# GDMCF/GDMCF

Hardware: AMD Instinct MI355X
Metric: training users/sec (higher is better)
Workload: dtype f32; 1 GPU; yelp-shape synthetic rows, batch=400/GPU, dims=[1000], T=5, noise_scale=0.01, linear-var, mean_type=x0, reweight, AdamW lr=1e-5 (BASELINE configs[1]); n_items=34395, global_batch=400, parallelism=dp1, batch_rows=device CSR rows (CsrBatch)

## Files before the change

### gdmcf_amd/csrc/gemm_dr.h

```cpp
#pragma once

#include "common.h"

namespace {
struct DrArgs {
    GdGemm g;
    int tiles_m, tiles_n, m_fastest;
    int ksp;
    int ctr;
    const GdAdamHyper* adam_dev;
    int stagger;
};
}

struct DrRoutes {
    bool dw;
    bool adamw;
    bool kn;
    bool fat;
    bool fat_slab;
};
DrRoutes& dr_routes();
int dr_cu_count();
int dr_stagger();

int gd_dr_tn_launch(GdGemm& g, hipStream_t s);
int gd_dr_kn_launch(GdGemm& g, hipStream_t s);
int gd_dr_fat_launch(int epi, GdGemm& g, hipStream_t s);
int gd_dr_fat_slab_launch(GdGemm& g, hipStream_t s);
```

### gdmcf_amd/csrc/gemm_dr_fat.hip

```cpp
#include <stdlib.h>

#include "gemm_dr.h"

#ifndef GD_FAT_DMA_DEFAULT
#define GD_FAT_DMA_DEFAULT 1
#endif

namespace {

template <int NB, int EPI, int DMA>
__global__ __launch_bounds__(256, 1) void dr_fat_kernel(const DrArgs d) {
    static_assert(EPI == GD_EPI_LOSS || EPI == GD_EPI_POST || EPI == GD_EPI_SLAB, "output layer with a fused epilogue, or split-K slabs");
    static_assert(NB >= 4 && NB <= 12, "5 x NB accumulator blocks must fit 256 registers");
    static_assert(DMA == 0 || DMA == 1, "B through staging registers, or straight into LDS");
    constexpr bool SLAB = EPI == GD_EPI_SLAB;
    typedef __attribute__((address_space(3))) void* lds_vp;
    constexpr int WAIT_VM0 = 0x0F70, WAIT_LGKM0 = 0xC07F;
    constexpr int TMB = 5;
    const GdGemm& g = d.g;
    const int lane = threadIdx.x & 63;
    const int wave = __builtin_amdgcn_readfirstlane(threadIdx.x >> 6);
    const int r = lane & 15, q = lane >> 4;
    extern __shared__ __attribute__((aligned(16))) float dr_lds[];
    float* const lds = dr_lds + wave * (2 * NB * 256);
    const int nblk = gridDim.x, per = nblk >> 3;
    const int wl = ((nblk & 7) == 0 ? ((int)(blockIdx.x & 7) * per + (int)(blockIdx.x >> 3)) : (int)blockIdx.x) * 4 + wave;
    const int n_waves = nblk * 4;
    const int ntiles = d.tiles_m * d.tiles_n;
    const __amdgpu_buffer_rsrc_t srdA = __builtin_amdgcn_make_buffer_rsrc(const_cast<float*>(g.A), 0, (int)(((int64_t)(g.M - 1) * g.lda + g.K) * 4), 0x00020000);
    const __amdgpu_buffer_rsrc_t srdB = __builtin_amdgcn_make_buffer_rsrc(const_cast<float*>(g.B), 0, (int)(((int64_t)(g.N - 1) * g.ldb + g.K) * 4), 0x00020000);
    const int NCH = d.ksp;
    const int c_mask = g.K >> 4;
    const int ntasks = SLAB ? ntiles * g.splits : ntiles;
    const int w_off = (lane >> 2) * 16 + (((lane & 3) ^ ((((lane >> 2) >> 2) & 1) << 1)) << 2);
    const int g_slot = DMA ? ((lane & 3) ^ ((((lane >> 2) >> 2) & 1) << 1)) : (lane & 3);
    const int r_off = r * 16 + ((q ^ (((r >> 2) & 1) << 1)) << 2);
    for (int task = wl; task < ntasks; task += n_waves) {
        const int split = SLAB ? task / ntiles : 0;
        const int tile = SLAB ? task - split * ntiles : task;
        const int c_lo = SLAB ? split * (g.kchunk >> 4) : 0;
        const int c_hi = SLAB ? min(c_lo + (g.kchunk >> 4), NCH) : NCH;
        const int c_in = SLAB ? min(c_hi, c_mask) : c_mask;
        const int tm = tile % d.tiles_m, tn = tile / d.tiles_m;
        const int m0 = tm * (16 * TMB), n0 = tn * (16 * NB);
        uint32_t offA[TMB], offB[NB];
#pragma unroll
        for (int i = 0; i < TMB; ++i) offA[i] = (uint32_t)((m0 + 16 * i + r) * g.lda + 4 * q) * 4u;
#pragma unroll
        for (int p = 0; p < NB; ++p) offB[p] = (uint32_t)(((int64_t)(n0 + 16 * p + (lane >> 2)) * g.ldb + 4 * g_slot) * 4);
        f32x4 acc[TMB][NB];
#pragma unroll
        for (int i = 0; i < TMB; ++i)
#pragma unroll
            for (int b = 0; b < NB; ++b) acc[i][b] = f32x4{0.f, 0.f, 0.f, 0.f};
        f32x4 xa[2][TMB], G[DMA ? 1 : NB], FB[NB];
        const int hp = DMA ? ((c_in - c_lo) & 1) : 0;
        const int k_lo = SLAB ? c_lo * 64 : 0;
        if (hp) {
#pragma unroll
            for (int i = 0; i < TMB; ++i) xa[1][i] = __builtin_bit_cast(f32x4, __builtin_amdgcn_raw_buffer_load_b128(srdA, offA[i], k_lo, 0));
        } else {
#pragma unroll
            for (int i = 0; i < TMB; ++i) xa[0][i] = __builtin_bit_cast(f32x4, __builtin_amdgcn_raw_buffer_load_b128(srdA, offA[i], k_lo, 0));
        }
        if constexpr (DMA) {
            __builtin_amdgcn_sched_barrier(0);
            __builtin_amdgcn_s_waitcnt(WAIT_LGKM0);
            __builtin_amdgcn_sched_barrier(0);
#pragma unroll
            for (int p = 0; p < NB; ++p) __builtin_amdgcn_raw_ptr_buffer_load_lds(srdB, (lds_vp)(lds + hp * (NB * 256) + p * 256), 16, (int)offB[p], k_lo, 0, 0);
        } else {
#pragma unroll
            for (int p = 0; p < NB; ++p) G[p] = __builtin_bit_cast(f32x4, __builtin_amdgcn_raw_buffer_load_b128(srdB, offB[p], k_lo, 0));
#pragma unroll
            for (int p = 0; p < NB; ++p) *reinterpret_cast<f32x4*>(lds + p * 256 + w_off) = G[p];
        }

#define GD_FAT_CHUNK(PAR, c, MSK)                                                                                         \
        {                                                                                                             \
             \
            const uint32_t kn = ((c) + 1 < c_hi) ? (uint32_t)((c) + 1) * 64u : 0x80000000u;                           \
            if constexpr (DMA) {                                                                                      \
                __builtin_amdgcn_sched_barrier(0);                                                                    \
                __builtin_amdgcn_s_waitcnt(WAIT_VM0);                                                                 \
                __builtin_amdgcn_sched_barrier(0);                                                                    \
            }                                                                                                         \
            _Pragma("unroll") for (int b = 0; b < NB; ++b)                                                            \
                FB[b] = *reinterpret_cast<const f32x4*>(lds + (PAR) * (NB * 256) + b * 256 + r_off);                  \
            if (MSK) {  \
                 \
                _Pragma("unroll") for (int e = 0; e < 4; ++e) {                                                       \
                    const bool keep = (c) * 16 + 4 * q + e < g.K;                                                     \
                    _Pragma("unroll") for (int i = 0; i < TMB; ++i) xa[PAR][i][e] = keep ? xa[PAR][i][e] : 0.f;       \
                    _Pragma("unroll") for (int b = 0; b < NB; ++b) FB[b][e] = keep ? FB[b][e] : 0.f;                  \
                }                                                                                                     \
            }                                                                                                         \
            __builtin_amdgcn_sched_barrier(0);                                                                        \
            _Pragma("unroll") for (int sx = 0; sx < 4; ++sx) {                                                        \
                _Pragma("unroll") for (int n = 0; n < TMB * NB; ++n) {                                                \
                    const int i = n / NB, b = n % NB;                                                                 \
                    if (sx == 0 && i == 0) asm volatile("" : "+v"(FB[b]));  \
                    if (sx == 0 && b == 0) asm volatile("" : "+v"(xa[PAR][i]));                                       \
                    acc[i][b] = __builtin_amdgcn_mfma_f32_16x16x4f32(xa[PAR][i][sx], FB[b][sx], acc[i][b], 0, 0, 0);  \
                     \
                    if (sx < 2 && n % 5 == 2) {      \
                        const int l = (sx == 0) ? n / 5 : NB + n / 5;                                                 \
                        if (l < TMB + NB) {                                                                           \
                            __builtin_amdgcn_sched_barrier(0);                                                        \
                            if (l < TMB)                                                                              \
                                xa[(PAR) ^ 1][l] = __builtin_bit_cast(f32x4, __builtin_amdgcn_raw_buffer_load_b128(   \
                                    srdA, offA[l], kn, 0));                                                           \
                            else if constexpr (DMA)                                                                   \
                                __builtin_amdgcn_raw_ptr_buffer_load_lds(                                             \
                                    srdB, (lds_vp)(lds + ((PAR) ^ 1) * (NB * 256) + (l - TMB) * 256), 16,             \
                                    (int)offB[l - TMB], (int)kn, 0, 0);                                               \
                            else                                                                                      \
                                G[l - TMB] = __builtin_bit_cast(f32x4, __builtin_amdgcn_raw_buffer_load_b128(         \
                                    srdB, offB[l - TMB], kn, 0));                                                     \
                            __builtin_amdgcn_sched_barrier(0);                                                        \
                        }                                                                                             \
                    }                                                                                                 \
                    if (!DMA && sx == 3 && n % 4 == 1 && n / 4 < NB) {  \
                        __builtin_amdgcn_sched_barrier(0);                                                            \
                        *reinterpret_cast<f32x4*>(lds + ((PAR) ^ 1) * (NB * 256) + (n / 4) * 256 + w_off) = G[n / 4]; \
                        __builtin_amdgcn_sched_barrier(0);                                                            \
                    }                                                                                                 \
                }                                                                                                     \
                __builtin_amdgcn_sched_barrier(0);                                                                    \
            }                                                                                                         \
        }
        const int c_pf = d.stagger > 0 ? ((NCH > d.stagger + 2 ? NCH - d.stagger : 0) & ~1) : -2;
        const int c_pairs = DMA ? c_in : c_hi;
        const int c_pfl = (DMA && c_pf >= 0) ? min(c_pf | hp, c_pairs - 2) : c_pf;
        int c = c_lo;
        if constexpr (DMA) {
            if (hp) {
                GD_FAT_CHUNK(1, c_lo, false);
                c = c_lo + 1;
            }
        }
        for (; c + 1 < c_pairs; c += 2) {
            if constexpr (EPI == GD_EPI_POST) {
                if (c == c_pfl) {
                    constexpr int NJL = (16 * NB * 4 + 127) / 128 + 1;
                    constexpr int NPI = (80 * NJL + 63) / 64;
                    float* const scratch = dr_lds + 4 * (2 * NB * 256) + wave * 64;
                    const __amdgpu_buffer_rsrc_t srdX = __builtin_amdgcn_make_buffer_rsrc(
                        const_cast<float*>(g.aux), 0, (int)(((int64_t)(g.M - 1) * g.ldaux + g.N) * 4), 0x00020000);
#pragma unroll
                    for (int pi = 0; pi < NPI; ++pi) {
                        const int t = min(pi * 64 + lane, 80 * NJL - 1);
                        const int row = min(m0 + t % 80, g.M - 1), j = t / 80;
                        const int col = min(j < NJL - 1 ? n0 + 32 * j : n0 + 16 * NB - 1, g.N - 1);
                        __builtin_amdgcn_raw_ptr_buffer_load_lds(srdX, (lds_vp)scratch, 4, (int)(((int64_t)row * g.ldaux + col) * 4), 0, 0, 0);
                    }
                }
            }
            if constexpr (DMA) {
                GD_FAT_CHUNK(0, c, false);
                GD_FAT_CHUNK(1, c + 1, false);
            } else {
                GD_FAT_CHUNK(0, c, c >= c_mask);
                GD_FAT_CHUNK(1, c + 1, c + 1 >= c_mask);
            }
        }
        if constexpr (DMA) {
            if (c < c_hi) GD_FAT_CHUNK(0, c, true);
        } else {
            if ((c_hi - c_lo) & 1) GD_FAT_CHUNK(0, c_hi - 1, c_hi - 1 >= c_mask);
        }
#undef GD_FAT_CHUNK
        if constexpr (DMA) {
            __builtin_amdgcn_sched_barrier(0);
            __builtin_amdgcn_s_waitcnt(WAIT_VM0);
            __builtin_amdgcn_sched_barrier(0);
        }

        if constexpr (SLAB) {
            constexpr int LDS_S = 16 * NB + 4, NJ_S = (4 * NB + 15) / 16;
            float* const slab = g.C + (int64_t)split * g.slab_stride;
#pragma unroll
            for (int i = 0; i < TMB; ++i) {
#pragma unroll
                for (int b = 0; b < NB; ++b)
#pragma unroll
                    for (int t = 0; t < 4; ++t) lds[(4 * q + t) * LDS_S + 16 * b + r] = acc[i][b][t];
                __builtin_amdgcn_sched_barrier(0);
#pragma unroll
                for (int p4 = 0; p4 < 4; ++p4) {
                    const int m = m0 + 16 * i + 4 * p4 + q;
#pragma unroll
                    for (int j = 0; j < NJ_S; ++j) {
                        const int c4 = r + 16 * j;
                        const int n = n0 + 4 * c4;
                        const f32x4 v = *reinterpret_cast<const f32x4*>(lds + (4 * p4 + q) * LDS_S + 4 * min(c4, 4 * NB - 1));
                        if (c4 < 4 * NB && m < g.M) {
                            if (n + 3 < g.N) {
                                *reinterpret_cast<f32x4*>(slab + (int64_t)m * g.ldc + n) = v;
                            } else {
                                for (int e = 0; e < 4 && n + e < g.N; ++e) slab[(int64_t)m * g.ldc + n + e] = v[e];
                            }
                        }
                    }
                }
                __builtin_amdgcn_sched_barrier(0);
            }
            continue;
        }

        constexpr int LDS_ = 16 * NB + 4;
        constexpr int NJ = (4 * NB + 15) / 16;
        typedef f32x4 f32x4_e __attribute__((aligned(4)));
        f32x4 bias4[NJ];
        int col4[NJ];
#pragma unroll
        for (int j = 0; j < NJ; ++j) {
            col4[j] = n0 + 4 * (r + 16 * j);
            bias4[j] = f32x4{0.f, 0.f, 0.f, 0.f};
            if (g.bias && r + 16 * j < 4 * NB) {
#pragma unroll
                for (int e = 0; e < 4; ++e) bias4[j][e] = g.bias[min(col4[j] + e, g.N - 1)];
            }
        }
        const bool has_z = (EPI == GD_EPI_POST) && (g.aux2 != nullptr);
        const bool has_r = (EPI == GD_EPI_POST) && (g.r2 != nullptr);
        struct Pre {
            f32x4 a[NJ], z[NJ];
            uint32_t w[NJ];
            float c1, c2, p1, p2, sg;
        } pre[2];
        auto fetch = [&](int i, int p4, Pre& P) {
            const int mc = min(m0 + 16 * i + 4 * p4 + q, g.M - 1);
            P.c1 = 1.f; P.c2 = 0.f; P.p1 = 0.f; P.p2 = 0.f; P.sg = 0.f;
            if (EPI == GD_EPI_LOSS) {
                if (g.r0) P.c1 = g.r0[mc];
            } else {
                P.c1 = g.r0[mc];
                P.c2 = g.r1[mc];
                if (has_r) { P.p1 = g.r2[mc]; P.p2 = g.r3[mc]; }
                if (has_z) P.sg = g.r4[mc];
            }
#pragma unroll
            for (int j = 0; j < NJ; ++j) {
                const int n = col4[j];
                const bool whole = (r + 16 * j < 4 * NB) && n + 3 < g.N;
                P.w[j] = 0u;
                P.a[j] = f32x4{0.f, 0.f, 0.f, 0.f};
                P.z[j] = f32x4{0.f, 0.f, 0.f, 0.f};
                if (EPI == GD_EPI_LOSS && g.aux_bits) {
                    P.w[j] = g.aux_bits[(int64_t)mc * g.ldbits + min((int64_t)(n >> 5), g.ldbits - 1)];
                } else if (whole) {
                    P.a[j] = *reinterpret_cast<const f32x4_e*>(g.aux + (int64_t)mc * g.ldaux + n);
                    if (has_z) P.z[j] = *reinterpret_cast<const f32x4_e*>(g.aux2 + (int64_t)mc * g.ldaux2 + n);
                }
            }
        };
        fetch(0, 0, pre[0]);
#pragma unroll
        for (int i = 0; i < TMB; ++i) {
#pragma unroll
            for (int b = 0; b < NB; ++b)
#pragma unroll
                for (int t = 0; t < 4; ++t) lds[(4 * q + t) * LDS_ + 16 * b + r] = acc[i][b][t];
            __builtin_amdgcn_sched_barrier(0);
#pragma unroll
            for (int p4 = 0; p4 < 4; ++p4) {
                const int step = 4 * i + p4;
                const Pre& P = pre[step & 1];
                if (step + 1 < 4 * TMB) fetch((step + 1) >> 2, (step + 1) & 3, pre[(step + 1) & 1]);
                const int m = m0 + 16 * i + 4 * p4 + q;
                const int mc = min(m, g.M - 1);
                const bool mok = m < g.M;
                float ss = 0.f;
                const float c1 = P.c1, c2 = P.c2, p1 = P.p1, p2 = P.p2, sg = P.sg;
#pragma unroll
                for (int j = 0; j < NJ; ++j) {
                    const int c4 = r + 16 * j;
                    const bool inb = c4 < 4 * NB;
                    const int n = col4[j];
                    const bool whole = inb && n + 3 < g.N;
                    const bool full = whole && mok;
                    const f32x4 v = *reinterpret_cast<const f32x4*>(lds + (4 * p4 + q) * LDS_ + 4 * min(c4, 4 * NB - 1));
                    f32x4 o, o2 = f32x4{0.f, 0.f, 0.f, 0.f};
                    if (EPI == GD_EPI_LOSS) {
                        f32x4 tg;
                        if (g.aux_bits) {
                            const uint32_t w = P.w[j] >> (n & 31);
#pragma unroll
                            for (int e = 0; e < 4; ++e) tg[e] = (float)((w >> e) & 1u);
                        } else if (whole) {
                            tg = P.a[j];
                        } else {
#pragma unroll
                            for (int e = 0; e < 4; ++e) tg[e] = g.aux[(int64_t)mc * g.ldaux + min(n + e, g.N - 1)];
                        }
#pragma unroll
                        for (int e = 0; e < 4; ++e) {
                            o2[e] = v[e] + bias4[j][e];
                            o[e] = c1 * o2[e] - tg[e];
                            if (inb && mok && n + e < g.N) ss += o[e] * o[e];
                        }
                    } else {
                        f32x4 xt = P.a[j], zz = P.z[j];
                        if (!whole) {
#pragma unroll
                            for (int e = 0; e < 4; ++e) {
                                xt[e] = g.aux[(int64_t)mc * g.ldaux + min(n + e, g.N - 1)];
                                if (has_z) zz[e] = g.aux2[(int64_t)mc * g.ldaux2 + min(n + e, g.N - 1)];
                            }
                        }
#pragma unroll
                        for (int e = 0; e < 4; ++e) {
                            const float vv = v[e] + bias4[j][e];
                            o2[e] = has_r ? (p1 * xt[e] - p2 * vv) : vv;
                            o[e] = c1 * o2[e] + c2 * xt[e];
                            if (has_z) o[e] += sg * zz[e];
                        }
                    }
                    if (full) {
                        *reinterpret_cast<f32x4_e*>(g.C + (int64_t)m * g.ldc + n) = o;
                        if (g.out2) *reinterpret_cast<f32x4_e*>(g.out2 + (int64_t)m * g.ldout2 + n) = o2;
                    } else if (inb && mok) {
                        for (int e = 0; e < 4 && n + e < g.N; ++e) {
                            g.C[(int64_t)m * g.ldc + n + e] = o[e];
                            if (g.out2) g.out2[(int64_t)m * g.ldout2 + n + e] = o2[e];
                        }
                    }
                }
                if (EPI == GD_EPI_LOSS) {
                    ss += __shfl_xor(ss, 1);
                    ss += __shfl_xor(ss, 2);
                    ss += __shfl_xor(ss, 4);
                    ss += __shfl_xor(ss, 8);
                    if (r == 0 && mok) g.rowpart[(int64_t)m * g.ld_rowpart + tn] = ss;
                }
                __builtin_amdgcn_sched_barrier(0);
            }
        }
    }
}

template <int NB>
int dr_fat_go(const DrArgs& d, int epi, int dma, int n_cu, hipStream_t s) {
    const size_t lds = (size_t)4 * 2 * NB * 256 * sizeof(float) + 4 * 64 * sizeof(float);
    void (*kern)(const DrArgs) =
        dma ? (epi == GD_EPI_SLAB ? dr_fat_kernel<NB, GD_EPI_SLAB, 1> : epi == GD_EPI_LOSS ? dr_fat_kernel<NB, GD_EPI_LOSS, 1> : dr_fat_kernel<NB, GD_EPI_POST, 1>)
            : (epi == GD_EPI_SLAB ? dr_fat_kernel<NB, GD_EPI_SLAB, 0> : epi == GD_EPI_LOSS ? dr_fat_kernel<NB, GD_EPI_LOSS, 0> : dr_fat_kernel<NB, GD_EPI_POST, 0>);
    static bool attr_set[6] = {false, false, false, false, false, false};
    const int ai = epi == GD_EPI_SLAB ? 4 + dma : 2 * dma + (epi == GD_EPI_LOSS);
    if (!attr_set[ai] && lds > 48 * 1024) {
        hipError_t e = hipFuncSetAttribute(reinterpret_cast<const void*>(kern), hipFuncAttributeMaxDynamicSharedMemorySize, (int)lds);
        if (e != hipSuccess) {
            gdmcf_set_error("hipFuncSetAttribute(dr_fat_kernel, LDS=%zu): %s", lds, hipGetErrorString(e));
            return GDMCF_E_HIP;
        }
        attr_set[ai] = true;
    }
    hipLaunchKernelGGL(kern, dim3(n_cu), dim3(256), lds, s, d);
    return GDMCF_OK;
}

int dr_fat_dma(const GdGemm& g) {
    static const int dma_env = getenv("GDMCF_FAT_DMA") ? atoi(getenv("GDMCF_FAT_DMA")) : GD_FAT_DMA_DEFAULT;
    return (dma_env > 0 && (reinterpret_cast<uintptr_t>(g.B) & 15) == 0 && (g.ldb & 3) == 0) ? 1 : 0;
}

}

int gd_dr_fat_launch(int epi, GdGemm& g, hipStream_t s) {
    if (!dr_routes().fat) return GD_DR_NOT_TAKEN;
    const int64_t lim = (int64_t)1 << 32;
    const int n_cu = dr_cu_count();
    const int tiles_m = gd_cdiv(g.M, 80);
    bool ok = (int64_t)g.M * g.lda * 4 < ((int64_t)1 << 31) && (int64_t)g.N * g.ldb * 4 < lim && g.lda >= g.K && g.ldb >= g.K &&
              g.K >= 256 && (long)tiles_m * 80 * 100 <= (long)g.M * 112 &&
              (n_cu & 7) == 0 && !(epi == GD_EPI_LOSS && g.rowpart == nullptr) &&
              !(epi == GD_EPI_LOSS && g.aux_bits && g.ldbits < (g.N + 31) / 32);
    int nb = 0;
    long best = 1L << 60;
    const long slots = 4L * n_cu;
    for (int c = 12; c >= 8 && ok; --c) {
        const long t = (long)tiles_m * gd_cdiv(g.N, 16 * c);
        const long cost = ((t + slots - 1) / slots) * c;
        if (t >= slots / 2 && cost < best) { best = cost; nb = c; }
    }
    if (ok && epi == GD_EPI_POST) {
        const long t128 = (long)gd_cdiv(g.M, 80) * gd_cdiv(g.N, 128);
        const long rounds = (t128 + 2 * n_cu - 1) / (2 * n_cu);
        if (t128 * 100 >= rounds * 2 * n_cu * 90) ok = false;
    }
    if (!ok || !nb || (epi == GD_EPI_LOSS && g.ld_rowpart < gd_cdiv(g.N, 16 * nb))) return GD_DR_NOT_TAKEN;
    DrArgs d = {};
    d.tiles_m = tiles_m;
    d.tiles_n = gd_cdiv(g.N, 16 * nb);
    d.m_fastest = 1;
    d.ksp = gd_cdiv(g.K, 16);
    {
        static const int pf = getenv("GDMCF_FAT_PF") ? atoi(getenv("GDMCF_FAT_PF")) : 10;
        d.stagger = pf;
    }
    const int dma = dr_fat_dma(g);
    g.tiles_m = d.tiles_m;
    g.tiles_n = d.tiles_n;
    d.g = g;
    d.ctr = 0;
    int rc = GDMCF_OK;
    {
        GdProfScope prof(g.prof_tag, 2.0 * g.M * g.N * g.K, s);
        switch (nb) {
            case 8: rc = dr_fat_go<8>(d, epi, dma, n_cu, s); break;
            case 9: rc = dr_fat_go<9>(d, epi, dma, n_cu, s); break;
            case 10: rc = dr_fat_go<10>(d, epi, dma, n_cu, s); break;
            case 11: rc = dr_fat_go<11>(d, epi, dma, n_cu, s); break;
            default: rc = dr_fat_go<12>(d, epi, dma, n_cu, s); break;
        }
    }
    if (rc != GDMCF_OK) return rc;
    t_gd_last_gemm = 4;
    return gd_launch_status("gemm_dr");
}

int gd_dr_fat_slab_plan(int M, int N, int K, int* nb_out, int* cps_out) {
    if (!dr_routes().fat_slab || M <= 0 || N < 128 || K < 4096) return 0;
    const int n_cu = dr_cu_count();
    const int tiles_m = gd_cdiv(M, 80);
    if ((n_cu & 7) != 0 || (long)tiles_m * 80 * 100 > (long)M * 112) return 0;
    const long slots = 4L * n_cu;
    const int chunks = gd_cdiv(K, 16);
    int nb = 0, cps = 0;
    long best = 1L << 60;
    for (int c = 8; c <= 12; ++c) {
        const long tiles = (long)tiles_m * gd_cdiv(N, 16 * c);
        if (tiles > slots) continue;
        long sp = slots / tiles;
        if (sp > chunks / 8) sp = chunks / 8;
        if (sp > 64) sp = 64;
        if (sp < 2) continue;
        const int per = gd_cdiv(chunks, (int)sp);
        if ((long)c * per < best) { best = (long)c * per; nb = c; cps = per; }
    }
    if (!nb) return 0;
    if (nb_out) *nb_out = nb;
    if (cps_out) *cps_out = cps;
    return gd_cdiv(chunks, cps);
}

int gd_dr_fat_slab_launch(GdGemm& g, hipStream_t s) {
    int nb = 0, cps = 0;
    const int splits = gd_dr_fat_slab_plan(g.M, g.N, g.K, &nb, &cps);
    if (!splits) return GD_DR_NOT_TAKEN;
    const size_t need = (size_t)splits * g.M * g.ldc * sizeof(float);
    const bool ok = gd_aligned16(g.C) && (g.ldc & 3) == 0 && g.ldc >= g.N &&
                    g.ws_cap >= need && g.slab_stride >= (int64_t)g.M * g.ldc && (g.slab_stride & 3) == 0 &&
                    (int64_t)g.M * g.lda * 4 < ((int64_t)1 << 31) && (int64_t)g.N * g.ldb * 4 < ((int64_t)1 << 32) && g.lda >= g.K && g.ldb >= g.K;
    if (!ok) return GD_DR_NOT_TAKEN;
    const int n_cu = dr_cu_count();
    DrArgs d = {};
    d.tiles_m = gd_cdiv(g.M, 80);
    d.tiles_n = gd_cdiv(g.N, 16 * nb);
    d.m_fastest = 1;
    d.ksp = gd_cdiv(g.K, 16);
    g.splits = splits;
    g.kchunk = cps * 16;
    g.tiles_m = d.tiles_m;
    g.tiles_n = d.tiles_n;
    d.g = g;
    d.ctr = 0;
    const int dma = dr_fat_dma(g);
    int rc = GDMCF_OK;
    {
        GdProfScope prof(g.prof_tag, 2.0 * g.M * g.N * g.K, s);
        switch (nb) {
            case 8: rc = dr_fat_go<8>(d, GD_EPI_SLAB, dma, n_cu, s); break;
            case 9: rc = dr_fat_go<9>(d, GD_EPI_SLAB, dma, n_cu, s); break;
            case 10: rc = dr_fat_go<10>(d, GD_EPI_SLAB, dma, n_cu, s); break;
            case 11: rc = dr_fat_go<11>(d, GD_EPI_SLAB, dma, n_cu, s); break;
            default: rc = dr_fat_go<12>(d, GD_EPI_SLAB, dma, n_cu, s); break;
        }
    }
    if (rc != GDMCF_OK) return rc;
    t_gd_last_gemm = 6;
    return gd_launch_status("gemm_dr_fat_slab");
}
```

Before: 322,500 users/s.

## Add lean buffer-load epilogue variants to the fat output-layer GEMM kernel

Adds a specialized epilogue for the fat GEMM's fused loss and post-processing outputs. It reads the GdGemm fields from the kernarg segment, uses raw buffer loads and stores with out-of-range parking offsets in place of branches and bounds clamps, and increments offsets by strides. The aim is to cut scalar and vector instruction overhead, register pressure and divergent guarded stores in the epilogue, which runs after the 34k-wide output GEMM. It adds template instantiations per variant, a special path for the ragged last column tile, 32-bit offset limits checked on the host, and debug switches.

```diff
diff --git a/gdmcf_amd/csrc/gemm_dr.h b/gdmcf_amd/csrc/gemm_dr.h
--- a/gdmcf_amd/csrc/gemm_dr.h
+++ b/gdmcf_amd/csrc/gemm_dr.h
@@ -24,6 +24,7 @@
 int dr_cu_count();
 int dr_stagger();
 
+
 int gd_dr_tn_launch(GdGemm& g, hipStream_t s);
 int gd_dr_kn_launch(GdGemm& g, hipStream_t s);
 int gd_dr_fat_launch(int epi, GdGemm& g, hipStream_t s);
diff --git a/gdmcf_amd/csrc/gemm_dr_fat.hip b/gdmcf_amd/csrc/gemm_dr_fat.hip
--- a/gdmcf_amd/csrc/gemm_dr_fat.hip
+++ b/gdmcf_amd/csrc/gemm_dr_fat.hip
@@ -5,12 +5,235 @@
 #ifndef GD_FAT_DMA_DEFAULT
 #define GD_FAT_DMA_DEFAULT 1
 #endif
+#ifndef GD_FAT_EPI_DEFAULT
+#define GD_FAT_EPI_DEFAULT 1
+#endif
+#ifndef GD_FAT_EPI_DBG
+#define GD_FAT_EPI_DBG 0
+#endif
 
 namespace {
 
-template <int NB, int EPI, int DMA>
+template <int NB, int EPI, int VAR>
+__device__ __forceinline__ void dr_fat_lean_epilogue(f32x4 (&acc)[5][NB], float* const lds, const int m0, const int n0, const int tn,
+                                                     const bool last_tn, int r, int q) {
+#pragma clang fp contract(off)
+    static_assert(offsetof(DrArgs, g) == 0, "the lean epilogue finds its GdGemm at offset 0 of the kernel-argument segment");
+    typedef const __attribute__((address_space(4))) DrArgs* kargs_p;
+    kargs_p ka = (kargs_p)__builtin_amdgcn_kernarg_segment_ptr();
+    asm volatile("" : "+s"(ka), "+v"(r), "+v"(q));
+    const __attribute__((address_space(4))) GdGemm& g = ka->g;
+    constexpr int TMB = 5, LDS_ = 16 * NB + 4, NJ = (4 * NB + 15) / 16;
+    constexpr bool LOSS = EPI == GD_EPI_LOSS, BITS = LOSS && VAR == 1, GEN = !LOSS && VAR == 2;
+    constexpr bool NO_ST = (GD_FAT_EPI_DBG & 2) != 0;
+    constexpr uint32_t PARK = 0x80000000u;
+    typedef uint32_t u32x4 __attribute__((ext_vector_type(4)));
+    auto srd = [](const void* p, int64_t bytes) {
+        return __builtin_amdgcn_make_buffer_rsrc(const_cast<void*>(p), 0, p ? (int)bytes : 0, 0x00020000);
+    };
+    auto ld1 = [](__amdgpu_buffer_rsrc_t s, uint32_t off) { return __builtin_amdgcn_raw_buffer_load_b32(s, (int)off, 0, 0); };
+    auto ld1f = [](__amdgpu_buffer_rsrc_t s, uint32_t off) { return __builtin_bit_cast(float, __builtin_amdgcn_raw_buffer_load_b32(s, (int)off, 0, 0)); };
+    auto ld4f = [](__amdgpu_buffer_rsrc_t s, uint32_t off) { return __builtin_bit_cast(f32x4, __builtin_amdgcn_raw_buffer_load_b128(s, (int)off, 0, 0)); };
+    auto st1f = [](float v, __amdgpu_buffer_rsrc_t s, uint32_t off) { __builtin_amdgcn_raw_buffer_store_b32(__builtin_bit_cast(uint32_t, v), s, (int)off, 0, 0); };
+    auto st4f = [](f32x4 v, __amdgpu_buffer_rsrc_t s, uint32_t off) { __builtin_amdgcn_raw_buffer_store_b128(__builtin_bit_cast(u32x4, v), s, (int)off, 0, 0); };
+    const int M = g.M, N = g.N;
+    const bool has_o2 = g.out2 != nullptr;
+    const bool has_r = GEN && g.r2 != nullptr, has_z = GEN && g.aux2 != nullptr;
+    const __amdgpu_buffer_rsrc_t srdC = srd(NO_ST ? nullptr : g.C, ((int64_t)(M - 1) * g.ldc + N) * 4);
+    const __amdgpu_buffer_rsrc_t srdO = srd(NO_ST ? nullptr : g.out2, ((int64_t)(M - 1) * g.ldout2 + N) * 4);
+    const __amdgpu_buffer_rsrc_t srdP = srd(NO_ST || !LOSS ? nullptr : g.rowpart, ((int64_t)(M - 1) * g.ld_rowpart + g.tiles_n) * 4);
+    const __amdgpu_buffer_rsrc_t srdBias = srd(g.bias, (int64_t)N * 4);
+    const __amdgpu_buffer_rsrc_t srdR0 = srd(g.r0, (int64_t)M * 4);
+    const __amdgpu_buffer_rsrc_t srdR1 = srd(LOSS ? nullptr : g.r1, (int64_t)M * 4);
+    const __amdgpu_buffer_rsrc_t srdR2 = srd(has_r ? g.r2 : nullptr, (int64_t)M * 4);
+    const __amdgpu_buffer_rsrc_t srdR3 = srd(has_r ? g.r3 : nullptr, (int64_t)M * 4);
+    const __amdgpu_buffer_rsrc_t srdR4 = srd(has_z ? g.r4 : nullptr, (int64_t)M * 4);
+    const __amdgpu_buffer_rsrc_t srdT = BITS ? srd(g.aux_bits, (int64_t)M * g.ldbits * 4) : srd(g.aux, ((int64_t)(M - 1) * g.ldaux + N) * 4);
+    const __amdgpu_buffer_rsrc_t srdZ = srd(has_z ? g.aux2 : nullptr, ((int64_t)(M - 1) * g.ldaux2 + N) * 4);
+
+    const uint32_t row = (uint32_t)(m0 + q), col = (uint32_t)(n0 + 4 * r);
+    uint32_t offC = (row * (uint32_t)g.ldc + col) * 4u, offO = (row * (uint32_t)g.ldout2 + col) * 4u;
+    uint32_t offP = (row * (uint32_t)g.ld_rowpart + (uint32_t)tn) * 4u;
+    uint32_t offT = BITS ? (row * (uint32_t)g.ldbits + (col >> 5)) * 4u : (row * (uint32_t)g.ldaux + col) * 4u;
+    uint32_t offZ = (row * (uint32_t)g.ldaux2 + col) * 4u;
+    const uint32_t strC = (uint32_t)g.ldc * 16u, strO = (uint32_t)g.ldout2 * 16u, strP = (uint32_t)g.ld_rowpart * 16u;
+    const uint32_t strT = (BITS ? (uint32_t)g.ldbits : (uint32_t)g.ldaux) * 16u, strZ = (uint32_t)g.ldaux2 * 16u;
+    const uint32_t offR = row * 4u;
+    const uint32_t sh = col & 31u;
+    bool gok[NJ];
+    f32x4 bias4[NJ];
+#pragma unroll
+    for (int j = 0; j < NJ; ++j) {
+        gok[j] = (r + 16 * j < 4 * NB) && (n0 + 4 * (r + 16 * j) + 3 < N);
+        bias4[j] = ld4f(srdBias, (gok[j] ? col * 4u : PARK) + 256u * j);
+    }
+    const bool sedge = last_tn && (N & 3) != 0;
+    const int c4s = sedge ? ((N - 1 - n0) >> 2) : 0;
+    const int ne = N & 3;
+    const uint32_t ns = (uint32_t)(n0 + 4 * c4s);
+    const bool sl = sedge && r == (c4s & 15);
+    const uint32_t dCs = (ns - col) * 4u;
+    const uint32_t dTs = BITS ? ((ns >> 5) - (col >> 5)) * 4u : dCs;
+    uint32_t parkS[3], dE[3];
+    float bs[3] = {0.f, 0.f, 0.f};
+#pragma unroll
+    for (int e = 0; e < 3; ++e) {
+        parkS[e] = (sl && e < ne) ? 0u : PARK;
+        dE[e] = 4u * (uint32_t)min(e, max(ne - 1, 0));
+    }
+    if (sedge) {
+#pragma unroll
+        for (int e = 0; e < 3; ++e) bs[e] = ld1f(srdBias, ns * 4u + dE[e]);
+    }
+
+    struct Pre {
+        f32x4 a[NJ], z[NJ];
+        uint32_t w[NJ], ws;
+        float c1, c2, p1, p2, sg, sa[3], sz[3];
+    } pre[2];
+    auto fetch = [&](const int step, Pre& P) {
+        const uint32_t oR = offR + 16u * step;
+        if constexpr (LOSS) {
+            const float c = ld1f(srdR0, oR);
+            P.c1 = g.r0 ? c : 1.f;
+        } else {
+            P.c1 = ld1f(srdR0, oR);
+            P.c2 = ld1f(srdR1, oR);
+            if constexpr (GEN) {
+                P.p1 = ld1f(srdR2, oR);
+                P.p2 = ld1f(srdR3, oR);
+                P.sg = ld1f(srdR4, oR);
+            }
+        }
+#pragma unroll
+        for (int j = 0; j < NJ; ++j) {
+            if constexpr (BITS) {
+                P.w[j] = ld1(srdT, offT + 8u * j);
+            } else {
+                P.a[j] = ld4f(srdT, (gok[j] ? offT : PARK) + 256u * j);
+                if constexpr (GEN) P.z[j] = ld4f(srdZ, (gok[j] ? offZ : PARK) + 256u * j);
+            }
+        }
+        if (sedge) {
+            if constexpr (BITS) {
+                P.ws = ld1(srdT, offT + dTs);
+            } else {
+#pragma unroll
+                for (int e = 0; e < 3; ++e) {
+                    P.sa[e] = ld1f(srdT, offT + dTs + dE[e]);
+                    if constexpr (GEN) P.sz[e] = ld1f(srdZ, offZ + dCs + dE[e]);
+                }
+            }
+        }
+    };
+    auto elem = [&](const Pre& P, float v, float b, float t, float z, float& o2, float& o) {
+        const float vv = v + b;
+        if constexpr (LOSS) {
+            o2 = vv;
+            o = __builtin_fmaf(P.c1, vv, -t);
+        } else {
+            o2 = vv;
+            if constexpr (GEN) {
+                const float e0 = P.p1 * t, e1 = P.p2 * vv;
+                o2 = has_r ? e0 - e1 : vv;
+            }
+            const float c = P.c1 * o2;
+            o = __builtin_fmaf(P.c2, t, c);
+            if constexpr (GEN) o = has_z ? __builtin_fmaf(P.sg, z, o) : o;
+        }
+    };
+    fetch(0, pre[0]);
+#pragma unroll
+    for (int i = 0; i < TMB; ++i) {
+#pragma unroll
+        for (int b = 0; b < NB; ++b)
+#pragma unroll
+            for (int t = 0; t < 4; ++t) lds[(4 * q + t) * LDS_ + 16 * b + r] = acc[i][b][t];
+        __builtin_amdgcn_sched_barrier(0);
+#pragma unroll
+        for (int p4 = 0; p4 < 4; ++p4) {
+            const int step = 4 * i + p4;
+            const Pre& P = pre[step & 1];
+            if (step + 1 < 4 * TMB) {
+                offT += strT;
+                if constexpr (GEN) offZ += strZ;
+                fetch(step + 1, pre[(step + 1) & 1]);
+            }
+            const float* const lrow = lds + (4 * p4 + q) * LDS_;
+            float ss = 0.f;
+            f32x4 o2s[NJ];
+#pragma unroll
+            for (int j = 0; j < NJ; ++j) {
+                const f32x4 v = *reinterpret_cast<const f32x4*>(lrow + 4 * r + 64 * j);
+                f32x4 t, z = f32x4{0.f, 0.f, 0.f, 0.f}, o;
+                if constexpr (BITS) {
+                    const uint32_t w = P.w[j] >> sh;
+#pragma unroll
+                    for (int e = 0; e < 4; ++e) t[e] = (float)((w >> e) & 1u);
+                } else {
+                    t = P.a[j];
+                    if constexpr (GEN) z = P.z[j];
+                }
+                float s2 = ss;
+#pragma unroll
+                for (int e = 0; e < 4; ++e) {
+                    float o2e, oe;
+                    elem(P, v[e], bias4[j][e], t[e], z[e], o2e, oe);
+                    o2s[j][e] = o2e;
+                    o[e] = oe;
+                    if constexpr (LOSS) {
+                        const float sq = oe * oe;
+                        s2 = s2 + sq;
+                    }
+                }
+                if constexpr (LOSS) ss = gok[j] ? s2 : ss;
+                st4f(o, srdC, (gok[j] ? offC : PARK) + 256u * j);
+            }
+            if (has_o2) {
+#pragma unroll
+                for (int j = 0; j < NJ; ++j) st4f(o2s[j], srdO, (gok[j] ? offO : PARK) + 256u * j);
+            }
+            if (sedge) {
+                const f32x4 v = *reinterpret_cast<const f32x4*>(lrow + 4 * c4s);
+                float s2 = ss;
+#pragma unroll
+                for (int e = 0; e < 3; ++e) {
+                    float t, z = 0.f, o2, o;
+                    if constexpr (BITS) {
+                        t = (float)((P.ws >> ((ns & 31u) + e)) & 1u);
+                    } else {
+                        t = P.sa[e];
+                        if constexpr (GEN) z = P.sz[e];
+                    }
+                    elem(P, v[e], bs[e], t, z, o2, o);
+                    if constexpr (LOSS) {
+                        const float sq = o * o;
+                        s2 = (e < ne) ? s2 + sq : s2;
+                    }
+                    st1f(o, srdC, (offC + dCs + 4u * e) | parkS[e]);
+                    if (has_o2) st1f(o2, srdO, (offO + dCs + 4u * e) | parkS[e]);
+                }
+                if constexpr (LOSS) ss = sl ? s2 : ss;
+            }
+            if constexpr (LOSS) {
+                ss += __shfl_xor(ss, 1);
+                ss += __shfl_xor(ss, 2);
+                ss += __shfl_xor(ss, 4);
+                ss += __shfl_xor(ss, 8);
+                st1f(ss, srdP, r == 0 ? offP : PARK);
+                offP += strP;
+            }
+            offC += strC;
+            offO += strO;
+            __builtin_amdgcn_sched_barrier(0);
+        }
+    }
+}
+
+template <int NB, int EPI, int DMA, int VAR>
 __global__ __launch_bounds__(256, 1) void dr_fat_kernel(const DrArgs d) {
     static_assert(EPI == GD_EPI_LOSS || EPI == GD_EPI_POST || EPI == GD_EPI_SLAB, "output layer with a fused epilogue, or split-K slabs");
+    static_assert(VAR >= 0 && VAR <= 2 && (VAR == 0 || EPI != GD_EPI_SLAB), "the lean epilogues are the fused ones'");
     static_assert(NB >= 4 && NB <= 12, "5 x NB accumulator blocks must fit 256 registers");
     static_assert(DMA == 0 || DMA == 1, "B through staging registers, or straight into LDS");
     constexpr bool SLAB = EPI == GD_EPI_SLAB;
@@ -207,6 +430,17 @@
             }
             continue;
         }
+        if constexpr ((GD_FAT_EPI_DBG & 1) != 0) {
+#pragma unroll
+            for (int i = 0; i < TMB; ++i)
+#pragma unroll
+                for (int b = 0; b < NB; ++b) asm volatile("" ::"a"(acc[i][b]));
+            continue;
+        }
+        if constexpr (VAR != 0) {
+            dr_fat_lean_epilogue<NB, EPI, VAR>(acc, lds, m0, n0, tn, tn == d.tiles_n - 1, r, q);
+            continue;
+        }
 
         constexpr int LDS_ = 16 * NB + 4;
         constexpr int NJ = (4 * NB + 15) / 16;
@@ -222,6 +456,7 @@
                 for (int e = 0; e < 4; ++e) bias4[j][e] = g.bias[min(col4[j] + e, g.N - 1)];
             }
         }
+        const bool dbg_st = (GD_FAT_EPI_DBG & 2) ? g.M < 0 : true;
         const bool has_z = (EPI == GD_EPI_POST) && (g.aux2 != nullptr);
         const bool has_r = (EPI == GD_EPI_POST) && (g.r2 != nullptr);
         struct Pre {
@@ -279,7 +514,7 @@
                     const bool inb = c4 < 4 * NB;
                     const int n = col4[j];
                     const bool whole = inb && n + 3 < g.N;
-                    const bool full = whole && mok;
+                    const bool full = whole && mok && dbg_st;
                     const f32x4 v = *reinterpret_cast<const f32x4*>(lds + (4 * p4 + q) * LDS_ + 4 * min(c4, 4 * NB - 1));
                     f32x4 o, o2 = f32x4{0.f, 0.f, 0.f, 0.f};
                     if (EPI == GD_EPI_LOSS) {
@@ -320,7 +555,7 @@
                     if (full) {
                         *reinterpret_cast<f32x4_e*>(g.C + (int64_t)m * g.ldc + n) = o;
                         if (g.out2) *reinterpret_cast<f32x4_e*>(g.out2 + (int64_t)m * g.ldout2 + n) = o2;
-                    } else if (inb && mok) {
+                    } else if (inb && mok && dbg_st) {
                         for (int e = 0; e < 4 && n + e < g.N; ++e) {
                             g.C[(int64_t)m * g.ldc + n + e] = o[e];
                             if (g.out2) g.out2[(int64_t)m * g.ldout2 + n + e] = o2[e];
@@ -332,7 +567,7 @@
                     ss += __shfl_xor(ss, 2);
                     ss += __shfl_xor(ss, 4);
                     ss += __shfl_xor(ss, 8);
-                    if (r == 0 && mok) g.rowpart[(int64_t)m * g.ld_rowpart + tn] = ss;
+                    if (r == 0 && mok && dbg_st) g.rowpart[(int64_t)m * g.ld_rowpart + tn] = ss;
                 }
                 __builtin_amdgcn_sched_barrier(0);
             }
@@ -340,14 +575,25 @@
     }
 }
 
+template <int NB, int EPI>
+void (*dr_fat_pick(int dma, int var))(const DrArgs) {
+    if constexpr (EPI == GD_EPI_SLAB) {
+        return dma ? dr_fat_kernel<NB, EPI, 1, 0> : dr_fat_kernel<NB, EPI, 0, 0>;
+    } else {
+        if (var == 1) return dma ? dr_fat_kernel<NB, EPI, 1, 1> : dr_fat_kernel<NB, EPI, 0, 1>;
+        if (var == 2) return dma ? dr_fat_kernel<NB, EPI, 1, 2> : dr_fat_kernel<NB, EPI, 0, 2>;
+        return dma ? dr_fat_kernel<NB, EPI, 1, 0> : dr_fat_kernel<NB, EPI, 0, 0>;
+    }
+}
+
 template <int NB>
-int dr_fat_go(const DrArgs& d, int epi, int dma, int n_cu, hipStream_t s) {
+int dr_fat_go(const DrArgs& d, int epi, int dma, int var, int n_cu, hipStream_t s) {
     const size_t lds = (size_t)4 * 2 * NB * 256 * sizeof(float) + 4 * 64 * sizeof(float);
-    void (*kern)(const DrArgs) =
-        dma ? (epi == GD_EPI_SLAB ? dr_fat_kernel<NB, GD_EPI_SLAB, 1> : epi == GD_EPI_LOSS ? dr_fat_kernel<NB, GD_EPI_LOSS, 1> : dr_fat_kernel<NB, GD_EPI_POST, 1>)
-            : (epi == GD_EPI_SLAB ? dr_fat_kernel<NB, GD_EPI_SLAB, 0> : epi == GD_EPI_LOSS ? dr_fat_kernel<NB, GD_EPI_LOSS, 0> : dr_fat_kernel<NB, GD_EPI_POST, 0>);
-    static bool attr_set[6] = {false, false, false, false, false, false};
-    const int ai = epi == GD_EPI_SLAB ? 4 + dma : 2 * dma + (epi == GD_EPI_LOSS);
+    void (*kern)(const DrArgs) = epi == GD_EPI_SLAB   ? dr_fat_pick<NB, GD_EPI_SLAB>(dma, 0)
+                                 : epi == GD_EPI_LOSS ? dr_fat_pick<NB, GD_EPI_LOSS>(dma, var)
+                                                      : dr_fat_pick<NB, GD_EPI_POST>(dma, var);
+    static bool attr_set[18] = {};
+    const int ai = ((epi == GD_EPI_SLAB ? 2 : epi == GD_EPI_LOSS ? 1 : 0) * 2 + dma) * 3 + var;
     if (!attr_set[ai] && lds > 48 * 1024) {
         hipError_t e = hipFuncSetAttribute(reinterpret_cast<const void*>(kern), hipFuncAttributeMaxDynamicSharedMemorySize, (int)lds);
         if (e != hipSuccess) {
@@ -363,6 +609,20 @@
 int dr_fat_dma(const GdGemm& g) {
     static const int dma_env = getenv("GDMCF_FAT_DMA") ? atoi(getenv("GDMCF_FAT_DMA")) : GD_FAT_DMA_DEFAULT;
     return (dma_env > 0 && (reinterpret_cast<uintptr_t>(g.B) & 15) == 0 && (g.ldb & 3) == 0) ? 1 : 0;
+}
+
+int dr_fat_epi_var(int epi, const GdGemm& g, int tiles_m) {
+    static const int epi_env = getenv("GDMCF_FAT_EPI") ? atoi(getenv("GDMCF_FAT_EPI")) : GD_FAT_EPI_DEFAULT;
+    if (epi_env <= 0) return 0;
+    const int64_t rows = (int64_t)tiles_m * 80, lim = (int64_t)1 << 31;
+    auto fits = [&](const void* p, int64_t ld) { return p == nullptr || (ld >= g.N && rows * ld * 4 < lim); };
+    bool ok = fits(g.C, g.ldc) && fits(g.out2, g.ldout2) && fits(g.aux2, g.ldaux2) && (int64_t)g.N * 4 < lim;
+    if (epi == GD_EPI_LOSS) {
+        ok = ok && rows * g.ld_rowpart * 4 < lim && (g.aux_bits ? rows * g.ldbits * 4 < lim : fits(g.aux, g.ldaux));
+        return !ok ? 0 : g.aux_bits ? 1 : 2;
+    }
+    ok = ok && fits(g.aux, g.ldaux);
+    return !ok ? 0 : (g.r2 || g.aux2) ? 2 : 1;
 }
 
 }
@@ -400,6 +660,7 @@
         d.stagger = pf;
     }
     const int dma = dr_fat_dma(g);
+    const int var = dr_fat_epi_var(epi, g, tiles_m);
     g.tiles_m = d.tiles_m;
     g.tiles_n = d.tiles_n;
     d.g = g;
@@ -408,11 +669,11 @@
     {
         GdProfScope prof(g.prof_tag, 2.0 * g.M * g.N * g.K, s);
         switch (nb) {
-            case 8: rc = dr_fat_go<8>(d, epi, dma, n_cu, s); break;
-            case 9: rc = dr_fat_go<9>(d, epi, dma, n_cu, s); break;
-            case 10: rc = dr_fat_go<10>(d, epi, dma, n_cu, s); break;
-            case 11: rc = dr_fat_go<11>(d, epi, dma, n_cu, s); break;
-            default: rc = dr_fat_go<12>(d, epi, dma, n_cu, s); break;
+            case 8: rc = dr_fat_go<8>(d, epi, dma, var, n_cu, s); break;
+            case 9: rc = dr_fat_go<9>(d, epi, dma, var, n_cu, s); break;
+            case 10: rc = dr_fat_go<10>(d, epi, dma, var, n_cu, s); break;
+            case 11: rc = dr_fat_go<11>(d, epi, dma, var, n_cu, s); break;
+            default: rc = dr_fat_go<12>(d, epi, dma, var, n_cu, s); break;
         }
     }
     if (rc != GDMCF_OK) return rc;
@@ -471,11 +732,11 @@
     {
         GdProfScope prof(g.prof_tag, 2.0 * g.M * g.N * g.K, s);
         switch (nb) {
-            case 8: rc = dr_fat_go<8>(d, GD_EPI_SLAB, dma, n_cu, s); break;
-            case 9: rc = dr_fat_go<9>(d, GD_EPI_SLAB, dma, n_cu, s); break;
-            case 10: rc = dr_fat_go<10>(d, GD_EPI_SLAB, dma, n_cu, s); break;
-            case 11: rc = dr_fat_go<11>(d, GD_EPI_SLAB, dma, n_cu, s); break;
-            default: rc = dr_fat_go<12>(d, GD_EPI_SLAB, dma, n_cu, s); break;
+            case 8: rc = dr_fat_go<8>(d, GD_EPI_SLAB, dma, 0, n_cu, s); break;
+            case 9: rc = dr_fat_go<9>(d, GD_EPI_SLAB, dma, 0, n_cu, s); break;
+            case 10: rc = dr_fat_go<10>(d, GD_EPI_SLAB, dma, 0, n_cu, s); break;
+            case 11: rc = dr_fat_go<11>(d, GD_EPI_SLAB, dma, 0, n_cu, s); break;
+            default: rc = dr_fat_go<12>(d, GD_EPI_SLAB, dma, 0, n_cu, s); break;
         }
     }
     if (rc != GDMCF_OK) return rc;
```

Result: no change. 325,500 users/s (median of 6 runs) (+0.9%).
